# One-2-3-45/One-2-3-45

Hardware: AMD Instinct MI355X
Metric: rays/sec + mesh-extract wall-clock per scene (8x256^2 views, 128^3 vol) (higher is better)
Workload: dtype f32 (matrix products as 3 f16 MFMAs on split operands, fp32 accumulate); 1 GPU; BASELINE config 2: 1 scene/GPU/step (a different seeded scene every step), 8 views 256x256, 128^3 volume, 262144 rays (64+64 samples), mesh grid 256^3; whole scene pass per step; views=8, volume=128, rays=262144, mesh_res=256, parallelism=scenes x1, precision=f16x3

## Files before the change

include/o2345.h:

```cpp
#ifndef O2345_H
#define O2345_H
#include <stddef.h>
#include <stdint.h>
#ifdef __cplusplus
extern "C" {
#endif

const char* o2345_last_error(void);
int o2345_version(void);
size_t o2345_render_io_size(void);
int o2345_render_io_layout(size_t* offsets_host, int n);
const char* o2345_knobs(void);

size_t o2345_costvol_workspace_bytes(int dx, int dy, int dz);
int o2345_costvol_index(const float* proj, int V, int H, int W, int dx, int dy, int dz, float voxel_size,
                        const float* origin_host, int min_views, uint8_t* cnt, int32_t* row_of_voxel, int32_t* coords,
                        int32_t* n_rows_dev, void* workspace, size_t workspace_bytes, void* stream);
int o2345_costvol_gather(const float* feats_nhwc, const float* proj, int V, int H, int W, int C, int dx, int dy, int dz,
                         float voxel_size, const float* origin_host, const uint8_t* cnt, const int32_t* coords,
                         int n_rows, float* out_rows, void* stream);
int o2345_nchw_to_nhwc(const float* in, float* out, int V, int C, int H, int W, void* stream);

int o2345_fpn_level(const float* fine, int c_in, const float* coarse, const float* weight, const float* bias, int V, int H, int W,
                    float* out, void* stream);
// ... 103 lines not shown
    float inv_s, alpha_inter_ratio, background;
    float weight_cull;
    float* mid_z; float* dists; float* pm; float* sdf; float* grad; float* rgb; uint8_t* nviews;
    float* color; float* depth; float* weights; float* cdf; float* weights_sum; float* weights_max; float* depth_var;
    float* alpha_sum; float* grad_err; uint8_t* color_mask;
    float* z_vals;
    float* scalars;
    unsigned long long* color_stats;
} O2345RenderIO;
size_t o2345_list_sort_workspace_bytes(long long n_max, int V);
int o2345_list_sort_by_visibility(const float* pts, const int32_t* list, const int32_t* count_dev, long long n_max, const float* proj, int V, int H, int W,
                                  int32_t* list_out, uint32_t* keys_out, void* workspace, size_t workspace_bytes, void* stream);
size_t o2345_render_workspace_bytes(int R, int n_samples, int n_importance, int V);
int o2345_render_rays(const O2345RenderIO* io, void* workspace, size_t workspace_bytes, void* stream);

int o2345_camera_terms(const float* intrinsics, const float* w2cs, int V, float* proj_out, float* cam_pos_out, void* stream);

int o2345_pack_color_maps(const float* feat_nchw, const float* color_nchw, int V, int H, int W, float* out_nhwc64,
                          void* stream);
int o2345_view_count(const float* pts, long long n, const float* maskvol, int D, const float* proj, int V, int H, int W,
                     uint8_t* out, void* stream);
int o2345_view_count_unlisted(const float* pts, long long n, const float* skip_if_positive, const float* maskvol, int D, const float* proj,
                              int V, int H, int W, uint8_t* out, void* stream);
int o2345_color_mfma_blob_floats(void);
int o2345_color_points_mfma(const float* blob, const float* vol_cl, const float* maskvol, int D, const float* cmaps,
                            const float* proj, const float* cam_pos, int V, int H, int W, const float* pts,
                            const int32_t* index, const int32_t* n_dev, long long n, const float* query_cam,
                            const float* normals, float* out_rgb, uint8_t* out_nviews, unsigned long long* stats_dev, void* stream);
int o2345_color_x3_blob_floats(void);
int o2345_color_points_x3(const float* blob, const float* vol_cl, const float* maskvol, int D, const float* cmaps,
                          const float* proj, const float* cam_pos, int V, int H, int W, const float* pts,
                          const int32_t* index, const int32_t* n_dev, long long n, const float* query_cam,
                          const float* normals, float* out_rgb, uint8_t* out_nviews, unsigned long long* stats_dev, void* stream);
int o2345_project_features(const float* vol_cl, const float* maskvol, int D, const float* cmaps, const float* proj, const float* cam_pos, int V,
                           int H, int W, const float* pts, long long P, const float* query_cam, const float* normals, float* geometry_feat,
                           float* rgb_feat, float* ray_diff, float* mask, void* stream);
int o2345_color_from_features(const float* blob, int x3, const float* geometry_feat, const float* rgb_feat, const float* ray_diff,
                              const float* mask, int V, long long P, float* out_rgb, uint8_t* out_nviews, void* stream);

size_t o2345_mc_workspace_bytes(int n0, int n1, int n2);
int o2345_marching_cubes_count(const float* u, int n0, int n1, int n2, double iso, void* workspace,
                               size_t workspace_bytes, long long* nv_host, long long* nt_host, void* stream);
int o2345_marching_cubes_emit(const float* u, int n0, int n1, int n2, double iso, void* workspace, double* verts,
                              void* tris, int index_bytes, void* stream);

size_t o2345_mesh_components_workspace_bytes(long long nv, long long nt);
int o2345_mesh_components_count(const void* tris, int index_bytes, long long nv, long long nt, long long min_faces, int keep_largest, void* workspace,
                                size_t workspace_bytes, int* labels, long long* n_components_host, long long* n_components_kept_host,
                                long long* nv_kept_host, long long* nt_kept_host, void* stream);
int o2345_mesh_components_emit(const double* verts, const void* tris, int index_bytes, long long nv, long long nt, void* workspace, double* verts_out,
                               void* tris_out, int* kept_out, void* stream);

size_t o2345_mesh_adjacency_workspace_bytes(long long nv, long long nt);
int o2345_mesh_adjacency_count(const void* tris, int index_bytes, long long nv, long long nt, void* workspace, size_t workspace_bytes,
                               long long* n_entries_host, void* stream);
int o2345_mesh_adjacency_emit(void* workspace, long long nv, int* offsets, int* neighbours, unsigned char* boundary, void* stream);
int o2345_mesh_smooth(const double* verts_in, long long nv, const int* offsets, const int* neighbours, const unsigned char* boundary_or_null, int iterations,
                      double lam, double mu, double* verts_tmp, double* verts_out, void* stream);

size_t o2345_mesh_decimate_workspace_bytes(long long nv, long long nt);
int o2345_mesh_decimate_count(const double* verts, const void* tris, int index_bytes, long long nv, long long nt, double cell, void* workspace,
                              size_t workspace_bytes, long long* n_clusters_host, long long* nv_out_host, long long* nt_out_host,
                              long long* n_degenerate_host, long long* n_duplicate_host, void* stream);
int o2345_mesh_decimate_emit(const double* verts, const void* tris, int index_bytes, long long nv, long long nt, void* workspace, double* verts_out,
                             void* tris_out, int* cluster, void* stream);

// ... 66 lines not shown
```

one-2-3-45_amd/csrc/api.cpp:

```cpp
#include <stdarg.h>
#include <stdio.h>
#include "common.h"

namespace o2345 {
static thread_local char g_err[512] = "";
void set_error(const char* fmt, ...) {
    va_list ap;
    va_start(ap, fmt);
    vsnprintf(g_err, sizeof g_err, fmt, ap);
    va_end(ap);
}
}

#include <stddef.h>

namespace o2345 {
int preload_costvol();
int preload_sparse();
int preload_sparse_mfma();
int preload_sdf_mlp();
int preload_sdf_mlp_x3();
int preload_render();
int preload_list_sort();
int preload_color_maps();
// ... 15 lines not shown
extern "C" {
const char* o2345_last_error(void) { return o2345::g_err; }
int o2345_version(void) { return 210; }

int o2345_preload(void) {
    int e, bad = 0;
    if ((e = o2345::preload_costvol())) bad = e;
    if ((e = o2345::preload_sparse())) bad = e;
    if ((e = o2345::preload_sparse_mfma())) bad = e;
    if ((e = o2345::preload_sdf_mlp())) bad = e;
    if ((e = o2345::preload_sdf_mlp_x3())) bad = e;
    if ((e = o2345::preload_render())) bad = e;
    if ((e = o2345::preload_list_sort())) bad = e;
    if ((e = o2345::preload_color_maps())) bad = e;
    if ((e = o2345::preload_color_pts())) bad = e;
    if ((e = o2345::preload_mcubes())) bad = e;
    if ((e = o2345::preload_mesh_components())) bad = e;
    if ((e = o2345::preload_mesh_smooth())) bad = e;
    if ((e = o2345::preload_mesh_decimate())) bad = e;
    if ((e = o2345::preload_mesh_project())) bad = e;
    if ((e = o2345::preload_mesh_pack())) bad = e;
    if ((e = o2345::preload_mesh_export())) bad = e;
    if ((e = o2345::preload_mesh_texture())) bad = e;
    if ((e = o2345::preload_mesh_distance())) bad = e;
    if ((e = o2345::preload_surface_trace())) bad = e;
    if ((e = o2345::preload_featmaps())) bad = e;
    if ((e = o2345::preload_convnet())) bad = e;
    O2345_REQUIRE(bad == 0, "preload: hipFuncGetAttributes failed (%s)", hipGetErrorString((hipError_t)bad));
    return 0;
}

const char* o2345_knobs(void) {
    static const struct Text { char s[160]; Text() { const o2345::Knobs& k = o2345::knobs();
        snprintf(s, sizeof s, "list_sort=%d sparse_brick=%d flat_sched=%d color_tiles=%d color_sched=%d ray_stream_min=%lld", k.list_sort, k.sparse_brick, k.flat_sched,
                 k.color_tiles, k.color_sched, k.ray_stream_min); } } t;
    return t.s;
}

size_t o2345_render_io_size(void) { return sizeof(O2345RenderIO); }
int o2345_render_io_layout(size_t* offsets_host, int n) {
#define F(name) offsetof(O2345RenderIO, name)
    static const size_t off[] = {
        F(sdf_blob), F(color_x3_blob), F(color_mfma_blob), F(vol_cl), F(maskvol), F(cmaps), F(proj), F(cam_pos), F(D), F(V), F(H), F(W),
        F(rays_o), F(rays_d), F(near_ray), F(far_ray), F(query_cam), F(t_rand), F(R), F(n_samples), F(n_importance), F(sdf_mode), F(segment_rays),
        F(near), F(far), F(sample_dist), F(inv_s), F(alpha_inter_ratio), F(background), F(weight_cull),
        F(mid_z), F(dists), F(pm), F(sdf), F(grad), F(rgb), F(nviews), F(color), F(depth), F(weights), F(cdf), F(weights_sum), F(weights_max),
        F(depth_var), F(alpha_sum), F(grad_err), F(color_mask), F(z_vals), F(scalars), F(color_stats)};
#undef F
    const int nf = (int)(sizeof off / sizeof off[0]);
    for (int i = 0; i < n && i < nf && offsets_host; ++i) offsets_host[i] = off[i];
    return nf;
}
}
```

one-2-3-45_amd/csrc/color_mfma.hip:

```cpp
#include "color_net.h"

namespace o2345 {

#ifdef O2345_TILES_KERNEL
template <int G, bool X3>
__global__ __launch_bounds__(768) void k_color_mfma(ColorMArgs a) {
    extern __shared__ __attribute__((aligned(16))) float lds[];
    constexpr int PPT = 32 / G;
    constexpr int OPV = 64 / G;
    constexpr int PST = 2 * 64 + 4;
    constexpr int SB = PPT * PST;
    constexpr int TOTAL = X3 ? CX_TOTAL : CM_TOTAL;
    constexpr int TAIL = X3 ? CX_A_END - CM_BIAS0 : 0;
    for (int i = threadIdx.x * 4; i < TOTAL; i += blockDim.x * 4)
        *reinterpret_cast<float4*>(lds + i) = *reinterpret_cast<const float4*>(a.blob + i);
    __syncthreads();
    const int lane = threadIdx.x & 63, j = lane & 31, h = lane >> 5, ptl = j / G, v = j % G;
    const int wave = threadIdx.x >> 6, nwave = blockDim.x >> 6;
    float* sbuf = lds + TOTAL + wave * SB;
    const long long n = a.n_dev ? (long long)*a.n_dev : a.n;
    const float m1 = X3 ? opaque_minus_one() : -1.f;
    const float s_abs = fabsf(lds[TAIL + CM_S]) * LOG2E;
    const int base_prio = (a.sched & 1) ? (wave >> 2) : 0;
    if (a.sched & 1) set_wave_prio(base_prio);
// ... 79 lines not shown
                for (int r = 0; r < 16; ++r) {
                    const int nidx = 32 * b + (r & 3) + 8 * (r >> 2) + 4 * h;
                    acc[b][r] += s0[nidx] + s0[64 + nidx];
                }
            __builtin_amdgcn_wave_barrier();
        }
        float score = view_network<X3>(acc, rf, g.rd, wgt, m, m1, lds, TAIL, lds + TAIL + CM_S, lane, h);
        if (m == 0.f) score = -1e9f;
        if (!view_ok) score = -INFINITY;
        const float smax = gmax<G>(score);
        const float ex = view_ok ? __builtin_amdgcn_exp2f(score - smax) : 0.f;
        const float bw = ex * crcp(gsum<G>(ex));
        const float bwn = bw * LN2;
        const float c0 = gsum<G>(rgb0 * bwn), c1 = gsum<G>(rgb1 * bwn), c2 = gsum<G>(rgb2 * bwn);
        const float nv = gsum<G>(m);
        if (live && v == 0 && h == 0) {
            a.out_rgb[3 * slot] = c0; a.out_rgb[3 * slot + 1] = c1; a.out_rgb[3 * slot + 2] = c2;
            if (a.out_nviews) a.out_nviews[slot] = (uint8_t)(nv + 0.5f);
        }
    }
}

#endif

}

using namespace o2345;

extern "C" {

int o2345_color_mfma_blob_floats(void) { return CM_TOTAL2; }
int o2345_color_x3_blob_floats(void) { return CX_TOTAL2; }

static int color_points(int x3, const float* blob, const float* vol_cl, const float* maskvol, int D, const float* cmaps, const float* proj,
                        const float* cam_pos, int V, int H, int W, const float* pts, const int32_t* index, const int32_t* n_dev, long long n,
                        const float* query_cam, const float* normals, float* out_rgb, uint8_t* out_nviews, unsigned long long* stats_dev, void* stream) {
    O2345_REQUIRE(blob && vol_cl && maskvol && cmaps && proj && cam_pos && pts && out_rgb, "color_points: null pointer");
    O2345_REQUIRE((query_cam != nullptr) != (normals != nullptr), "color_points: give exactly one of query_cam / normals");
    O2345_REQUIRE(V >= 1 && V <= 255, "color_points: V must be in [1,255] (valid-view counts are stored as uint8; got %d)", V);
    if (n <= 0 && !n_dev) return 0;
    ColorMArgs a{blob, vol_cl, maskvol, D, cmaps, proj, cam_pos, V, H, W, pts, index, n_dev, n, query_cam, normals, out_rgb, out_nviews};
    a.sched = color_sched_mode();
    a.stats = stats_dev;
#ifdef O2345_TILES_KERNEL
    if (knobs().color_tiles && V <= 32) {
        int G = 4;
        while (G < V) G <<= 1;
        const int threads = 768, ppt = 32 / G;
        const unsigned grid = network_grid(n, n_dev, threads, ppt);
        const size_t lds = (size_t)((x3 ? CX_TOTAL : CM_TOTAL) + (threads / 64) * ppt * (2 * 64 + 4)) * sizeof(float);
        hipStream_t s = (hipStream_t)stream;
#define O2345_CM_CASE(GG, XX)                                                                                              \
    if (G == GG && (x3 != 0) == XX) {                                                                                      \
        O2345_ENSURE_LDS((k_color_mfma<GG, XX>), lds);                                                                     \
        hipLaunchKernelGGL((k_color_mfma<GG, XX>), dim3(grid), dim3(threads), lds, s, a);                                  \
    }
        O2345_CM_CASE(4, false) O2345_CM_CASE(8, false) O2345_CM_CASE(16, false) O2345_CM_CASE(32, false)
        O2345_CM_CASE(4, true) O2345_CM_CASE(8, true) O2345_CM_CASE(16, true) O2345_CM_CASE(32, true)
#undef O2345_CM_CASE
        return check_launch("color_points (tiles kernel)");
    }
#endif
    return color_pts_launch(a, x3, false, "color_points (points-as-columns kernel)", stream);
}

int o2345_color_points_mfma(const float* blob, const float* vol_cl, const float* maskvol, int D, const float* cmaps,
                            const float* proj, const float* cam_pos, int V, int H, int W, const float* pts,
                            const int32_t* index, const int32_t* n_dev, long long n, const float* query_cam,
                            const float* normals, float* out_rgb, uint8_t* out_nviews, unsigned long long* stats_dev, void* stream) {
    return color_points(0, blob, vol_cl, maskvol, D, cmaps, proj, cam_pos, V, H, W, pts, index, n_dev, n, query_cam, normals, out_rgb, out_nviews, stats_dev, stream);
}
int o2345_color_points_x3(const float* blob, const float* vol_cl, const float* maskvol, int D, const float* cmaps,
                          const float* proj, const float* cam_pos, int V, int H, int W, const float* pts,
                          const int32_t* index, const int32_t* n_dev, long long n, const float* query_cam,
                          const float* normals, float* out_rgb, uint8_t* out_nviews, unsigned long long* stats_dev, void* stream) {
    return color_points(1, blob, vol_cl, maskvol, D, cmaps, proj, cam_pos, V, H, W, pts, index, n_dev, n, query_cam, normals, out_rgb, out_nviews, stats_dev, stream);
}

int o2345_project_features(const float* vol_cl, const float* maskvol, int D, const float* cmaps, const float* proj, const float* cam_pos, int V, int H,
                           int W, const float* pts, long long P, const float* query_cam, const float* normals, float* geometry_feat, float* rgb_feat,
                           float* ray_diff, float* mask, void* stream) {
    O2345_REQUIRE(vol_cl && maskvol && cmaps && proj && cam_pos && pts && geometry_feat && rgb_feat && ray_diff && mask, "project_features: null pointer");
    O2345_REQUIRE((query_cam != nullptr) != (normals != nullptr), "project_features: give exactly one of query_cam / normals");
    O2345_REQUIRE(V >= 1 && V <= 255 && P >= 0 && P * V < (1ll << 33), "project_features: bad sizes (V in [1,255])");
    if (P == 0) return 0;
    const ColorMArgs a{nullptr, vol_cl, maskvol, D, cmaps, proj, cam_pos, V, H, W, pts, nullptr, nullptr, P, query_cam, normals, nullptr, nullptr};
    return project_features_launch(a, geometry_feat, rgb_feat, ray_diff, mask, stream);
}

int o2345_color_from_features(const float* blob, int x3, const float* geometry_feat, const float* rgb_feat, const float* ray_diff, const float* mask,
                              int V, long long P, float* out_rgb, uint8_t* out_nviews, void* stream) {
    O2345_REQUIRE(blob && geometry_feat && rgb_feat && ray_diff && mask && out_rgb, "color_from_features: null pointer");
    O2345_REQUIRE(V >= 1 && V <= 255 && P >= 0, "color_from_features: bad sizes (V in [1,255]: valid-view counts are stored as uint8)");
    if (P == 0) return 0;
    ColorMArgs a{};
    a.blob = blob; a.V = V; a.n = P; a.out_rgb = out_rgb; a.out_nviews = out_nviews;
    a.f_geo = geometry_feat; a.f_rgb = rgb_feat; a.f_rdiff = ray_diff; a.f_mask = mask;
    return color_pts_launch(a, x3, true, "color_from_features", stream);
}

}
```

one-2-3-45_amd/csrc/color_net.h:

```cpp
#pragma once
#include "common.h"
#include "geom_math.h"
#include "split_f16.h"

namespace o2345 {

#define MFMA32(a, b, c) __builtin_amdgcn_mfma_f32_32x32x2f32((a), (b), (c), 0, 0, 0)

constexpr int CM_A_RD0 = 0;
constexpr int CM_A_RD1 = CM_A_RD0 + 1 * 2 * 64;
constexpr int CM_A_B0 = CM_A_RD1 + 2 * 8 * 64;
constexpr int CM_A_B1 = CM_A_B0 + 2 * 32 * 64;
constexpr int CM_A_V0 = CM_A_B1 + 32 * 64;
constexpr int CM_A_V1 = CM_A_V0 + 16 * 64;
constexpr int CM_A_V20 = CM_A_V1 + 16 * 64;
constexpr int CM_A_R0 = CM_A_V20 + 16 * 64;
constexpr int CM_A_R1 = CM_A_R0 + 19 * 64;
constexpr int CM_BIAS0 = CM_A_R1 + 8 * 64;
constexpr int CM_B_RD0 = CM_BIAS0, CM_B_RD1 = CM_B_RD0 + 32, CM_B_B0 = CM_B_RD1 + 64, CM_B_B1 = CM_B_B0 + 64,
              CM_B_V0 = CM_B_B1 + 32, CM_B_V1 = CM_B_V0 + 32, CM_B_V20 = CM_B_V1 + 32, CM_B_R0 = CM_B_V20 + 32,
              CM_B_R1 = CM_B_R0 + 32, CM_V_V1X = CM_B_R1 + 32, CM_V_V21 = CM_V_V1X + 32, CM_V_R2 = CM_V_V21 + 32;
constexpr int CM_W_S = CM_V_R2 + 32;
constexpr int CM_S = CM_W_S + 144 * 64;
constexpr int CM_TOTAL = CM_S + 4;
constexpr int CX_A_RD0 = 0;
constexpr int CX_A_RD1 = CX_A_RD0 + 1 * 1 * 512;
constexpr int CX_A_B0 = CX_A_RD1 + 2 * 1 * 512;
constexpr int CX_A_B1 = CX_A_B0 + 2 * 4 * 512;
constexpr int CX_A_V0 = CX_A_B1 + 4 * 512;
constexpr int CX_A_V1 = CX_A_V0 + 2 * 512;
constexpr int CX_A_V20 = CX_A_V1 + 2 * 512;
constexpr int CX_A_R0 = CX_A_V20 + 2 * 512;
constexpr int CX_A_R1 = CX_A_R0 + 3 * 512;
constexpr int CX_A_END = CX_A_R1 + 1 * 512;
constexpr int CX_TOTAL = CX_A_END + (CM_TOTAL - CM_BIAS0);
constexpr int CM_A_S = CM_TOTAL;
constexpr int CM_TOTAL2 = CM_A_S + 2 * 72 * 64;
constexpr int CX_A_S = CX_TOTAL;
constexpr int CX_TOTAL2 = CX_A_S + 2 * 9 * 512;

struct ColorMArgs {
    const float* blob;
    const float* vol_cl; const float* maskvol; int D;
    const float* cmaps; const float* proj; const float* cam_pos; int V, H, W_img;
    const float* pts; const int* index; const int* n_dev; long long n;
    const float* query_cam; const float* normals;
    float* out_rgb; uint8_t* out_nviews;
    const float* f_geo;
    const float* f_rgb;
    const float* f_rdiff;
    const float* f_mask;
    unsigned long long* stats;
    int sched;
};

inline int color_sched_mode() { return knobs().color_sched; }
#if defined(__HIPCC__)
__device__ __forceinline__ void set_wave_prio(int p) {
    switch (p) {
        case 0: __builtin_amdgcn_s_setprio(0); break;
        case 1: __builtin_amdgcn_s_setprio(1); break;
        case 2: __builtin_amdgcn_s_setprio(2); break;
        default: __builtin_amdgcn_s_setprio(3); break;
    }
}
#endif

constexpr float LOG2E = 1.44269504088896340736f, LN2 = 0.69314718055994530942f;
__device__ __forceinline__ float celu(float y) {
    const float t = __builtin_amdgcn_fmed3f(__builtin_amdgcn_exp2f(y), 0.f, 1.f);
    return fmaxf(y, fmaf(t, LOG2E, -LOG2E));
}
typedef float f32x2 __attribute__((ext_vector_type(2)));
__device__ __forceinline__ f32x2 celu2(float y0, float y1) {
    f32x2 t;
    t[0] = __builtin_amdgcn_fmed3f(__builtin_amdgcn_exp2f(y0), 0.f, 1.f);
    t[1] = __builtin_amdgcn_fmed3f(__builtin_amdgcn_exp2f(y1), 0.f, 1.f);
    const f32x2 e = __builtin_elementwise_fma(t, f32x2{LOG2E, LOG2E}, f32x2{-LOG2E, -LOG2E});
    return f32x2{fmaxf(y0, e[0]), fmaxf(y1, e[1])};
}
__device__ __forceinline__ float crcp(float x) { return __builtin_amdgcn_rcpf(x); }
__device__ __forceinline__ float csigm(float z) { return crcp(1.f + __builtin_amdgcn_exp2f(-z)); }

template <int NB, int NST, int N>
__device__ __forceinline__ void cm_run(f32x16 (&acc)[NB], const float* A , int step0, const float (&b)[N]) {
    float cur[NB], nxt[NB];
// ... 274 lines not shown
```

one-2-3-45_amd/csrc/color_pts.hip:

```cpp
#include "color_net.h"

namespace o2345 {

__device__ __forceinline__ ViewGeom feat_geom(const ColorMArgs& a, int v, long long slot, float s_abs) {
    ViewGeom g;
    const float4 rd = *reinterpret_cast<const float4*>(a.f_rdiff + ((size_t)v * a.n + slot) * 4);
    g.rd[0] = rd.x; g.rd[1] = rd.y; g.rd[2] = rd.z; g.rd[3] = rd.w;
    g.e = __builtin_amdgcn_exp2f(s_abs * (rd.w - 1.f));
    g.m = a.f_mask[(size_t)v * a.n + slot] != 0.f ? 1.f : 0.f;
    g.gx = g.gy = 0.f;
    return g;
}
__device__ __forceinline__ void load_feats(const ColorMArgs& a, int h, int v, long long slot, float (&rf)[32]) {
    const float* src = a.f_rgb + ((size_t)v * a.n + slot) * 59 + 32 * h;
#pragma unroll
    for (int c = 0; c < 32; ++c) rf[c] = (h == 0 || c < 27) ? src[(h == 0 || c < 27) ? c : 0] * LOG2E : 0.f;
}

template <bool FEATS>
__device__ __forceinline__ void pixel_floats(const ColorMArgs& a, int h, int v, long long slot, const ViewGeom& g, int base_prio, float (&rf)[32]) {
    if constexpr (FEATS) load_feats(a, h, v, slot, rf);
    else {
        if (a.sched & 2) set_wave_prio(3);
        gather_now(a, h, v, g, rf);
// ... 34 lines not shown
#pragma unroll
    for (int nb = 0; nb < NB; ++nb) cur[nb] = fetch(nb, 0);
#pragma unroll
    for (int r = 0; r < N; ++r) {
        if (r + 1 < N) {
#pragma unroll
            for (int nb = 0; nb < NB; ++nb) nxt[nb] = fetch(nb, r + 1);
        }
#pragma unroll
        for (int nb = 0; nb < NB; ++nb) acc[nb] = MFMA32(cur[nb], b[r], acc[nb]);
#pragma unroll
        for (int nb = 0; nb < NB; ++nb) cur[nb] = nxt[nb];
        __builtin_amdgcn_sched_barrier(0);
    }
}

__device__ __forceinline__ void sh_store(float4* slot, const f32x16 (&sh)[2]) {
#pragma unroll
    for (int nb = 0; nb < 2; ++nb)
#pragma unroll
        for (int q = 0; q < 4; ++q) slot[(nb * 4 + q) * 64] = make_float4(sh[nb][4 * q], sh[nb][4 * q + 1], sh[nb][4 * q + 2], sh[nb][4 * q + 3]);
}
__device__ __forceinline__ void sh_load(f32x16 (&acc)[2], const float4* slot) {
#pragma unroll
    for (int nb = 0; nb < 2; ++nb)
#pragma unroll
        for (int q = 0; q < 4; ++q) {
            const float4 t = slot[(nb * 4 + q) * 64];
            acc[nb][4 * q] = t.x; acc[nb][4 * q + 1] = t.y; acc[nb][4 * q + 2] = t.z; acc[nb][4 * q + 3] = t.w;
        }
}

constexpr int CP_THREADS = 768;
constexpr int CP_SH_FLOATS = 2 * 16 * 64;
constexpr size_t color_pts_lds_bytes(int x3) {
    return (size_t)((x3 ? CX_A_END + CM_W_S - CM_BIAS0 : CM_W_S) + 4 + (CP_THREADS / 64) * CP_SH_FLOATS) * sizeof(float);
}
static_assert(color_pts_lds_bytes(1) <= 160 * 1024 && color_pts_lds_bytes(0) <= 160 * 1024, "k_color_pts: LDS of a CU exceeded");
template <bool X3, bool FEATS>
__global__ __launch_bounds__(CP_THREADS) void k_color_pts(ColorMArgs a) {
    extern __shared__ __attribute__((aligned(16))) float lds[];
    constexpr int HEAD = X3 ? (CX_A_END + CM_W_S - CM_BIAS0) : CM_W_S;
    constexpr int SRC_S = X3 ? (CX_TOTAL - 4) : CM_S;
    constexpr int TAIL = X3 ? CX_A_END - CM_BIAS0 : 0;
    constexpr int L_S = HEAD, L_SH = HEAD + 4;
    for (int i = threadIdx.x * 4; i < HEAD; i += blockDim.x * 4)
        *reinterpret_cast<float4*>(lds + i) = *reinterpret_cast<const float4*>(a.blob + i);
    if (threadIdx.x == 0) *reinterpret_cast<float4*>(lds + L_S) = *reinterpret_cast<const float4*>(a.blob + SRC_S);
    __syncthreads();
    const int lane = threadIdx.x & 63, j = lane & 31, h = lane >> 5;
    const int wave = threadIdx.x >> 6, nwave = blockDim.x >> 6;
    float4* const sh_slot = reinterpret_cast<float4*>(lds + L_SH + wave * CP_SH_FLOATS) + lane;
    const long long n = a.n_dev ? (long long)*a.n_dev : a.n;
    const float m1 = X3 ? opaque_minus_one() : -1.f;
    const float s_abs = fabsf(lds[L_S]) * LOG2E;
    const int V = a.V;
    const bool skip_views = V <= 64 && !(a.sched & 4);
    const bool skip_zero = skip_views && !(a.sched & 16);
    const int base_prio = (a.sched & 1) ? (wave >> 2) : 0;
    if (a.sched & 1) set_wave_prio(base_prio);
    const TileSched ts = (a.sched & 8) ? TileSched{(long long)blockIdx.x * nwave + wave, (n + 31) / 32, (long long)gridDim.x * nwave}
                                       : tile_schedule(n, 32, wave, nwave);
    unsigned st_a = 0, st_b = 0, st_t = 0, st_full = 0;
    for (long long tile = ts.first; tile < ts.end; tile += ts.stride) {
        const long long i = tile * 32 + j;
        const bool live = i < n;
        const long long slot = live ? (a.index ? (long long)a.index[i] : i) : 0;
        const float px = (live && !FEATS) ? a.pts[3 * slot] : 0.f, py = (live && !FEATS) ? a.pts[3 * slot + 1] : 0.f,
                    pz = (live && !FEATS) ? a.pts[3 * slot + 2] : 0.f;
        float bs[72];
        bool gvalid;
        if constexpr (FEATS) {
            const float4* g4 = reinterpret_cast<const float4*>(a.f_geo + (size_t)slot * 16) + 2 * h;
            const float4 t0 = g4[0], t1 = g4[1];
            bs[0] = t0.x; bs[1] = t0.y; bs[2] = t0.z; bs[3] = t0.w; bs[4] = t1.x; bs[5] = t1.y; bs[6] = t1.z; bs[7] = t1.w;
            gvalid = true;
        } else {
#pragma unroll
            for (int c = 0; c < 8; ++c) bs[c] = 0.f;
            const float msum = trilinear_taps(px, py, pz, a.D, a.maskvol, [&](size_t vox, float w) {
                fma_rows<2>(reinterpret_cast<const float4*>(a.vol_cl + vox * 16) + 2 * h, w, bs);
            });
            gvalid = point_valid(px, py, pz, msum);
        }
        float qx = 0.f, qy = 0.f, qz = 0.f;
        if constexpr (!FEATS) query_direction(a.normals, a.query_cam, slot, px, py, pz, qx, qy, qz);
        float emin = INFINITY;
        for (int v = 0; v < V; ++v) {
            if constexpr (FEATS) {
                emin = fminf(emin, __builtin_amdgcn_exp2f(s_abs * (a.f_rdiff[((size_t)v * a.n + slot) * 4 + 3] - 1.f)));
                continue;
            }
            const float sx = a.cam_pos[3 * v] - px, sy = a.cam_pos[3 * v + 1] - py, sz = a.cam_pos[3 * v + 2] - pz;
            const float rsn = crcp(sqrtf(sx * sx + sy * sy + sz * sz) + 1e-6f);
            const float dot = qx * (sx * rsn) + qy * (sy * rsn) + qz * (sz * rsn);
            emin = fminf(emin, __builtin_amdgcn_exp2f(s_abs * (dot - 1.f)));
        }
// ... 151 lines not shown
```

one-2-3-45_amd/csrc/common.h:

```cpp
#pragma once
#include "../../include/o2345.h"
#include <atomic>
#include <cstdlib>
#include <hip/hip_runtime.h>
#include <stdint.h>
#include <stdio.h>

#define O2345_HD __host__ __device__ __forceinline__

namespace o2345 {

void set_error(const char* fmt, ...);

inline int check_launch(const char* what) {
    hipError_t e = hipGetLastError();
    if (e != hipSuccess) {
        set_error("%s: %s", what, hipGetErrorString(e));
        return -2;
    }
    return 0;
}

#define O2345_REQUIRE(cond, ...)            \
    do {                                    \
// ... 28 lines not shown

__device__ __forceinline__ int lane_id() { return __lane_id(); }

__device__ __forceinline__ int wave_prefix(bool pred, int& total) {
    unsigned long long m = __ballot(pred);
    total = __popcll(m);
    return __popcll(m & ((1ull << lane_id()) - 1ull));
}

template <int NWAVES>
__device__ __forceinline__ int block_prefix(bool pred, int* lds_wave_tot , int& block_total) {
    int wtot;
    int p = wave_prefix(pred, wtot);
    const int w = threadIdx.x >> 6;
    if (lane_id() == 0) lds_wave_tot[w] = wtot;
    __syncthreads();
    int base = 0, tot = 0;
#pragma unroll
    for (int i = 0; i < NWAVES; ++i) {
        int t = lds_wave_tot[i];
        if (i < w) base += t;
        tot += t;
    }
    block_total = tot;
    __syncthreads();
    return base + p;
}


struct Knobs {
    bool list_sort, sparse_brick, flat_sched, color_tiles;
    int color_sched;
    long long ray_stream_min;
};
inline const Knobs& knobs() {
    static const Knobs k = [] {
        auto is = [](const char* name, char c) { const char* e = getenv(name); return e && e[0] == c; };
        const char* cs = getenv("O2345_COLOR_SCHED");
        const char* rs = getenv("O2345_RAY_STREAM_MIN");
        return Knobs{!is("O2345_LIST_SORT", '0'), !is("O2345_SPARSE_BRICK", '0'), is("O2345_FLAT_SCHED", '1'), is("O2345_COLOR_KERNEL", 't'), cs ? atoi(cs) : 10,
                     rs ? atoll(rs) : 4096};
    }();
    return k;
}

struct MaxLds {
    std::atomic<int> cur[64];
    MaxLds() { for (auto& c : cur) c.store(0, std::memory_order_relaxed); }
    hipError_t ensure(const void* func, size_t bytes) {
        int dev = 0;
        if (hipGetDevice(&dev) != hipSuccess || dev < 0 || dev >= 64) return hipFuncSetAttribute(func, hipFuncAttributeMaxDynamicSharedMemorySize, (int)bytes);
        if ((int)bytes <= cur[dev].load(std::memory_order_acquire)) return hipSuccess;
        const hipError_t e = hipFuncSetAttribute(func, hipFuncAttributeMaxDynamicSharedMemorySize, (int)bytes);
        if (e == hipSuccess) cur[dev].store((int)bytes, std::memory_order_release);
        return e;
    }
};
#define O2345_ENSURE_LDS(kernel, bytes)                                                   \
    do {                                                                                  \
        static o2345::MaxLds max_lds_;                                                    \
        O2345_HIP(max_lds_.ensure((const void*)(kernel), (size_t)(bytes)));               \
    } while (0)

inline unsigned persistent_grid(long long want, int n_cu) {
    unsigned g = (unsigned)(want < n_cu ? want : n_cu);
    if (knobs().flat_sched && g > 8 && (g & 7) == 0) --g;
    return g;
}

inline unsigned network_grid(long long n, const void* n_dev, int threads, int units_per_wave) {
    const int n_cu = cu_count();
    const long long per_block = (long long)(threads / 64) * units_per_wave;
    return persistent_grid(n_dev ? n_cu : (n + per_block - 1) / per_block, n_cu);
}

#if defined(__HIPCC__)
struct TileSched { long long first, end, stride; };
__device__ __forceinline__ TileSched tile_schedule(long long n_units, int units_per_tile, int wave, int nwave) {
    const long long ntiles = (n_units + units_per_tile - 1) / units_per_tile;
    if ((gridDim.x & 7) == 0) {
        const int xcd = blockIdx.x & 7, slot = blockIdx.x >> 3, per_xcd = gridDim.x >> 3;
        const long long chunk = (ntiles + 7) / 8, lo = xcd * chunk, hi = lo + chunk;
        return {lo + (long long)slot * nwave + wave, hi < ntiles ? hi : ntiles, (long long)per_xcd * nwave};
    }
    return {(long long)blockIdx.x * nwave + wave, ntiles, (long long)gridDim.x * nwave};
}
#endif

}
```

one-2-3-45_amd/csrc/render.hip:

```cpp
#include "common.h"
#include "render_math.h"

namespace o2345 {

enum RenderCounter {
    RC_ROUND = 0,
    RC_FINAL = 4,
    RC_CULLED = 5,
    RC_DONE = 8,
    RC_CLEARED = 16,
    RC_RESERVED = 64
};

__global__ __launch_bounds__(256) void k_ray_coarse(RayGeom g, float near, float far, const float* __restrict__ near_ray,
                                                    const float* __restrict__ far_ray, int S, const float* __restrict__ t_rand,
                                                    float* __restrict__ z, float* __restrict__ pts, const float* __restrict__ maskvol, int D,
                                                    uint8_t* __restrict__ msk, int* __restrict__ counters) {
    if (counters && blockIdx.x == 0 && threadIdx.x < RC_CLEARED) counters[threadIdx.x] = 0;
    const long long p = (long long)blockIdx.x * 256 + threadIdx.x;
    if (p >= (long long)S * g.R) return;
    const int s = (int)(p / g.R), r = (int)(p % g.R);
    if (near_ray) { near = near_ray[r]; far = far_ray[r]; }
    float zz = near + (far - near) * linspace_at(0.f, 1.f, S, s);
    if (t_rand) {
        const float zp = near + (far - near) * linspace_at(0.f, 1.f, S, s > 0 ? s - 1 : 0);
        const float zn = near + (far - near) * linspace_at(0.f, 1.f, S, s < S - 1 ? s + 1 : S - 1);
        const float lower = s > 0 ? 0.5f * (zz + zp) : zz;
        const float upper = s < S - 1 ? 0.5f * (zn + zz) : zz;
        zz = lower + (upper - lower) * t_rand[(long long)r * S + s];
    }
    z[p] = zz;
    float x, y, w;
    ray_point(g, r, zz, x, y, w);
    pts[3 * p] = x; pts[3 * p + 1] = y; pts[3 * p + 2] = w;
    if (msk) msk[p] = mask_at(maskvol, D, x, y, w) > 0.f ? 1 : 0;
}

__device__ __forceinline__ unsigned long long lanes_below() { return (1ull << (threadIdx.x & 63)) - 1ull; }
__device__ __forceinline__ int reserve_slots(int* __restrict__ count, int n, int* __restrict__ seg_cnt, int ray0, int seg_rays) {
    const int base = atomicAdd(count, n);
    if (seg_cnt) atomicAdd(seg_cnt + ray0 / seg_rays, n);
    return base;
}
__device__ __forceinline__ void append_lane(bool valid, int slot, int* __restrict__ list, int* __restrict__ count, int* __restrict__ seg_cnt = nullptr,
                                            int ray0 = 0, int seg_rays = 0) {
// ... 752 lines not shown
    const bool sorts = render_sorts_list(R, NS, NIMP, io->V);
    int* slist = lay.at<int>(workspace, lay.sorted_list);
    auto sort_list = [&](const int* in, const int* n_dev) {
        return o2345_list_sort_by_visibility(fpts, in, n_dev, (long long)(S * RR), io->proj, io->V, io->H, io->W, slist, nullptr, lay.at<void>(workspace, lay.sort_ws),
                                             lay.sort_ws.bytes, stream);
    };
    const int* clist = list;
    const int* ccount = count;
    const float* counted_elsewhere = io->pm;
    if (!cull && sorts) {
        if ((rc = sort_list(list, count))) return rc;
        list = slist; clist = slist;
    }
    if ((rc = sdf_eval(2, fpts, list, count, 0, io->sdf, io->grad))) return rc;
    if (cull) {
        int* list2 = lay.at<int>(workspace, lay.cull_list);
        int* count2 = counters + RC_CULLED;
        float* keep = sdf;
        const size_t lds = group_lds_bytes(CULL_ARRAYS, (int)S);
        if (use_group_form(R, lds))
            hipLaunchKernelGGL(k_ray_cull_group, dim3(cdiv(R, GR)), dim3(64), lds, s, ra.g, (int)S, io->dists, io->pm, io->sdf, io->grad, io->inv_s, io->alpha_inter_ratio,
                               io->weight_cull, keep, io->rgb, list2, count2);
        else
            hipLaunchKernelGGL(k_ray_cull, dim3(cdiv(R, 256)), dim3(256), 0, s, ra.g, (int)S, io->dists, io->pm, io->sdf, io->grad, io->inv_s, io->alpha_inter_ratio,
                               io->weight_cull, keep, io->rgb, list2, count2);
        if ((rc = check_launch("ray_cull"))) return rc;
        clist = list2; ccount = count2; counted_elsewhere = keep;
        if (sorts) {
            if ((rc = sort_list(list2, count2))) return rc;
            clist = slist;
        }
    }
    if ((rc = o2345_view_count_unlisted(fpts, (long long)S * R, counted_elsewhere, io->maskvol, io->D, io->proj, io->V, io->H, io->W, io->nviews, stream))) return rc;
    const auto color_points = io->color_x3_blob ? o2345_color_points_x3 : o2345_color_points_mfma;
    rc = color_points(io->color_x3_blob ? io->color_x3_blob : io->color_mfma_blob, io->vol_cl, io->maskvol, io->D, io->cmaps, io->proj, io->cam_pos, io->V, io->H, io->W, fpts, clist,
                      ccount, 0, io->query_cam, nullptr, io->rgb, io->nviews, io->color_stats, stream);
    if (rc) return rc;
    if ((rc = o2345_ray_composite(io->rays_o, io->rays_d, R, (int)S, io->mid_z, io->dists, io->pm, io->sdf, io->grad, io->rgb, io->nviews, io->inv_s, io->alpha_inter_ratio, io->background,
                                  io->color, io->depth, io->weights, io->cdf, io->weights_sum, io->weights_max, io->depth_var, io->alpha_sum, io->grad_err, io->color_mask, stream))) return rc;
    if (io->scalars) hipLaunchKernelGGL(k_ray_scalars, dim3(G ? n_seg : 1), dim3(1024), 0, s, R, (int)S, io->alpha_sum, io->grad_err, G ? segc + (size_t)4 * n_seg : count,
                                        io->scalars, G);
    if (io->z_vals) O2345_HIP(hipMemcpyAsync(io->z_vals, z, S * RR * sizeof(float), hipMemcpyDeviceToDevice, s));
    return check_launch("render_rays");
}

}

namespace o2345 {
int preload_render() {
    hipFuncAttributes at;
    return (int)hipFuncGetAttributes(&at, (const void*)(k_quirk_min2));
}
}
```

one-2-3-45_amd/ops.py:

```python
import ctypes
import functools
from collections import namedtuple
import threading

import numpy as np
import torch

from . import _lib, config, mesh_io


call = _lib.call


def _first_cuda_tensor(objs):
    for o in objs:
        if torch.is_tensor(o):
            if o.is_cuda:
                return o
        elif isinstance(o, dict):
            t = _first_cuda_tensor(o.values())
            if t is not None:
                return t
    return None

# ... 396 lines not shown
             res.get("lat"), res.get("grad"))
    return res


def sdf_grid_active_points(device):
    with torch.cuda.device(device):
        ws = _workspace(None, torch.device(device), "sdf_grid_sparse")
    return None if ws is None else int(ws[:4].view(torch.int32).item())


@_on_device
def pack_color_maps(feat_nchw, color_nchw):
    V, _, H, W = feat_nchw.shape
    out = torch.empty(V, H, W, 64, dtype=torch.float32, device=feat_nchw.device)
    call("o2345_pack_color_maps", feat_nchw, color_nchw, V, H, W, out)
    return out


@_on_device
def camera_terms(intrinsics, w2cs):
    V = intrinsics.shape[0]
    if tuple(intrinsics.shape) != (V, 3, 3) or tuple(w2cs.shape) != (V, 4, 4):
        raise ValueError(f"camera_terms: intrinsics [V,3,3] and w2cs [V,4,4] expected, got {tuple(intrinsics.shape)}, {tuple(w2cs.shape)}")
    proj = torch.empty(V, 3, 4, dtype=torch.float32, device=w2cs.device)
    cam = torch.empty(V, 3, dtype=torch.float32, device=w2cs.device)
    call("o2345_camera_terms", _f(intrinsics), _f(w2cs), V, proj, cam)
    return proj, cam


def color_stats_buffer(device):
    return torch.zeros(4, dtype=torch.int64, device=device)


def color_stats_read(buf):
    out = [int(x) for x in buf.cpu().tolist()]
    return dict(pairs_pooling=out[0], pairs_network=out[1], tiles=out[2], tiles_all_views=out[3])


@_on_device
def color_points(blob, vol_cl, maskvol, cmaps, proj, cam_pos, pts, query_cam=None, normals=None, index=None, n_dev=None,
                 want_nviews=True, mfma="x3", stats=None):
    if mfma is False or mfma is None:
        raise ValueError("color_points: the pure-VALU colour kernel was removed in ABI 2.0; pass mfma='x3' (split-f16) or mfma=True (fp32 MFMA)")
    V, H, W, _ = cmaps.shape
    P = pts.shape[0]
    n = P if index is None else index.shape[0]
    rgb = torch.zeros(P, 3, dtype=torch.float32, device=pts.device)
    nv = torch.zeros(P, dtype=torch.uint8, device=pts.device) if want_nviews else None
    if P == 0 or (n == 0 and n_dev is None):
        return rgb, nv
    call("o2345_color_points_x3" if mfma == "x3" else "o2345_color_points_mfma", blob, vol_cl, maskvol, vol_cl.shape[0], cmaps, proj, cam_pos,
         V, H, W, pts, index, n_dev, n, query_cam, normals, rgb, nv, stats)
    return rgb, nv


@_on_device
def project_features(vol_cl, maskvol, cmaps, proj, cam_pos, pts, query_cam=None, normals=None):
    V, H, W, _ = cmaps.shape
    P = pts.shape[0]
    dev = pts.device
    geo = torch.empty(P, 16, dtype=torch.float32, device=dev)
    rf = torch.empty(V, P, 59, dtype=torch.float32, device=dev)
    rd = torch.empty(V, P, 4, dtype=torch.float32, device=dev)
    m = torch.empty(V, P, dtype=torch.float32, device=dev)
    call("o2345_project_features", vol_cl, maskvol, vol_cl.shape[0], cmaps, proj, cam_pos, V, H, W, pts, P, query_cam, normals, geo, rf, rd, m)
    return geo, rf, rd, m


@_on_device
def color_from_features(blob, geometry_feat, rgb_feat, ray_diff, mask, x3=True, want_nviews=True):
    V, P, C = rgb_feat.shape
    if C != 59 or tuple(geometry_feat.shape) != (P, 16) or tuple(ray_diff.shape) != (V, P, 4) or tuple(mask.shape) != (V, P):
        raise ValueError(f"color_from_features: expected geometry_feat [P,16], rgb_feat [V,P,59], ray_diff [V,P,4], mask [V,P]; got "
                         f"{tuple(geometry_feat.shape)}, {tuple(rgb_feat.shape)}, {tuple(ray_diff.shape)}, {tuple(mask.shape)}")
    rgb = torch.empty(P, 3, dtype=torch.float32, device=rgb_feat.device)
    nv = torch.empty(P, dtype=torch.uint8, device=rgb_feat.device) if want_nviews else None
    if P:
        call("o2345_color_from_features", blob, int(bool(x3)), _f(geometry_feat), _f(rgb_feat), _f(ray_diff), _f(mask), V, P, rgb, nv)
    return rgb, nv


@_on_device
def view_count(pts, maskvol, D, proj, V, H, W):
    out = torch.empty(pts.shape[0], dtype=torch.uint8, device=pts.device)
    call("o2345_view_count", pts, pts.shape[0], maskvol, D, proj, V, H, W, out)
# ... 688 lines not shown
```

Before: 4.680 million rays/s.

## Add atomic tile queue for dynamic load balancing in colour-points kernel

Adds a dynamic tile queue to the colour-points MFMA kernel. A fraction of the tiles is handed out from 8 per-XCD atomic heads instead of a fixed strided schedule. With the default share shift of 0, every tile is claimed dynamically. The queue heads live in the render counter block, which k_ray_coarse clears, and the queue is on by default through a new knob. The aim is to even out per-wave work when tiles differ in cost (views skipped, masked points), at the price of one atomic per tile and the loss of the static per-XCD chunking.

Result: faster. 4.903 million rays/s (median of 6 runs) (+4.8%).

```diff
diff --git a/include/o2345.h b/include/o2345.h
--- a/include/o2345.h
+++ b/include/o2345.h
@@ -159,6 +159,14 @@
                           const float* proj, const float* cam_pos, int V, int H, int W, const float* pts,
                           const int32_t* index, const int32_t* n_dev, long long n, const float* query_cam,
                           const float* normals, float* out_rgb, uint8_t* out_nviews, unsigned long long* stats_dev, void* stream);
+int o2345_color_points_mfma_q(const float* blob, const float* vol_cl, const float* maskvol, int D, const float* cmaps,
+                              const float* proj, const float* cam_pos, int V, int H, int W, const float* pts,
+                              const int32_t* index, const int32_t* n_dev, long long n, const float* query_cam,
+                              const float* normals, float* out_rgb, uint8_t* out_nviews, unsigned long long* stats_dev, int32_t* tile_queue, void* stream);
+int o2345_color_points_x3_q(const float* blob, const float* vol_cl, const float* maskvol, int D, const float* cmaps,
+                            const float* proj, const float* cam_pos, int V, int H, int W, const float* pts,
+                            const int32_t* index, const int32_t* n_dev, long long n, const float* query_cam,
+                            const float* normals, float* out_rgb, uint8_t* out_nviews, unsigned long long* stats_dev, int32_t* tile_queue, void* stream);
 int o2345_project_features(const float* vol_cl, const float* maskvol, int D, const float* cmaps, const float* proj, const float* cam_pos, int V,
                            int H, int W, const float* pts, long long P, const float* query_cam, const float* normals, float* geometry_feat,
                            float* rgb_feat, float* ray_diff, float* mask, void* stream);
diff --git a/one-2-3-45_amd/csrc/api.cpp b/one-2-3-45_amd/csrc/api.cpp
--- a/one-2-3-45_amd/csrc/api.cpp
+++ b/one-2-3-45_amd/csrc/api.cpp
@@ -71,8 +71,8 @@
 
 const char* o2345_knobs(void) {
     static const struct Text { char s[160]; Text() { const o2345::Knobs& k = o2345::knobs();
-        snprintf(s, sizeof s, "list_sort=%d sparse_brick=%d flat_sched=%d color_tiles=%d color_sched=%d ray_stream_min=%lld", k.list_sort, k.sparse_brick, k.flat_sched,
-                 k.color_tiles, k.color_sched, k.ray_stream_min); } } t;
+        snprintf(s, sizeof s, "list_sort=%d sparse_brick=%d flat_sched=%d color_tiles=%d color_sched=%d ray_stream_min=%lld tile_queue=%d", k.list_sort, k.sparse_brick,
+                 k.flat_sched, k.color_tiles, k.color_sched, k.ray_stream_min, k.tile_queue); } } t;
     return t.s;
 }
 
diff --git a/one-2-3-45_amd/csrc/color_mfma.hip b/one-2-3-45_amd/csrc/color_mfma.hip
--- a/one-2-3-45_amd/csrc/color_mfma.hip
+++ b/one-2-3-45_amd/csrc/color_mfma.hip
@@ -135,16 +135,21 @@
 int o2345_color_mfma_blob_floats(void) { return CM_TOTAL2; }
 int o2345_color_x3_blob_floats(void) { return CX_TOTAL2; }
 
-static int color_points(int x3, const float* blob, const float* vol_cl, const float* maskvol, int D, const float* cmaps, const float* proj,
-                        const float* cam_pos, int V, int H, int W, const float* pts, const int32_t* index, const int32_t* n_dev, long long n,
-                        const float* query_cam, const float* normals, float* out_rgb, uint8_t* out_nviews, unsigned long long* stats_dev, void* stream) {
+}
+
+int o2345::color_points_launch(int x3, const float* blob, const float* vol_cl, const float* maskvol, int D, const float* cmaps, const float* proj,
+                               const float* cam_pos, int V, int H, int W, const float* pts, const int32_t* index, const int32_t* n_dev, long long n,
+                               const float* query_cam, const float* normals, float* out_rgb, uint8_t* out_nviews, unsigned long long* stats_dev,
+                               int32_t* tile_queue, void* stream) {
     O2345_REQUIRE(blob && vol_cl && maskvol && cmaps && proj && cam_pos && pts && out_rgb, "color_points: null pointer");
     O2345_REQUIRE((query_cam != nullptr) != (normals != nullptr), "color_points: give exactly one of query_cam / normals");
     O2345_REQUIRE(V >= 1 && V <= 255, "color_points: V must be in [1,255] (valid-view counts are stored as uint8; got %d)", V);
     if (n <= 0 && !n_dev) return 0;
+    O2345_REQUIRE(!tile_queue || n <= TQ_MAX_TILES * 32, "color_points: a tile queue indexes at most %lld tiles", TQ_MAX_TILES);
     ColorMArgs a{blob, vol_cl, maskvol, D, cmaps, proj, cam_pos, V, H, W, pts, index, n_dev, n, query_cam, normals, out_rgb, out_nviews};
     a.sched = color_sched_mode();
     a.stats = stats_dev;
+    a.tile_queue = tile_queue;
 #ifdef O2345_TILES_KERNEL
     if (knobs().color_tiles && V <= 32) {
         int G = 4;
@@ -167,17 +172,43 @@
     return color_pts_launch(a, x3, false, "color_points (points-as-columns kernel)", stream);
 }
 
+extern "C" {
+
+static int color_points_q(int x3, const float* blob, const float* vol_cl, const float* maskvol, int D, const float* cmaps, const float* proj,
+                          const float* cam_pos, int V, int H, int W, const float* pts, const int32_t* index, const int32_t* n_dev, long long n,
+                          const float* query_cam, const float* normals, float* out_rgb, uint8_t* out_nviews, unsigned long long* stats_dev,
+                          int32_t* tile_queue, void* stream) {
+    O2345_REQUIRE(tile_queue, "color_points_q: null tile queue");
+    O2345_HIP(hipMemsetAsync(tile_queue, 0, TQ_HEADS * sizeof(int32_t), (hipStream_t)stream));
+    return color_points_launch(x3, blob, vol_cl, maskvol, D, cmaps, proj, cam_pos, V, H, W, pts, index, n_dev, n, query_cam, normals, out_rgb, out_nviews, stats_dev,
+                               tile_queue, stream);
+}
+int o2345_color_points_x3_q(const float* blob, const float* vol_cl, const float* maskvol, int D, const float* cmaps,
+                            const float* proj, const float* cam_pos, int V, int H, int W, const float* pts,
+                            const int32_t* index, const int32_t* n_dev, long long n, const float* query_cam,
+                            const float* normals, float* out_rgb, uint8_t* out_nviews, unsigned long long* stats_dev, int32_t* tile_queue, void* stream) {
+    return color_points_q(1, blob, vol_cl, maskvol, D, cmaps, proj, cam_pos, V, H, W, pts, index, n_dev, n, query_cam, normals, out_rgb, out_nviews, stats_dev,
+                          tile_queue, stream);
+}
+int o2345_color_points_mfma_q(const float* blob, const float* vol_cl, const float* maskvol, int D, const float* cmaps,
+                              const float* proj, const float* cam_pos, int V, int H, int W, const float* pts,
+                              const int32_t* index, const int32_t* n_dev, long long n, const float* query_cam,
+                              const float* normals, float* out_rgb, uint8_t* out_nviews, unsigned long long* stats_dev, int32_t* tile_queue, void* stream) {
+    return color_points_q(0, blob, vol_cl, maskvol, D, cmaps, proj, cam_pos, V, H, W, pts, index, n_dev, n, query_cam, normals, out_rgb, out_nviews, stats_dev,
+                          tile_queue, stream);
+}
+
 int o2345_color_points_mfma(const float* blob, const float* vol_cl, const float* maskvol, int D, const float* cmaps,
                             const float* proj, const float* cam_pos, int V, int H, int W, const float* pts,
                             const int32_t* index, const int32_t* n_dev, long long n, const float* query_cam,
                             const float* normals, float* out_rgb, uint8_t* out_nviews, unsigned long long* stats_dev, void* stream) {
-    return color_points(0, blob, vol_cl, maskvol, D, cmaps, proj, cam_pos, V, H, W, pts, index, n_dev, n, query_cam, normals, out_rgb, out_nviews, stats_dev, stream);
+    return color_points_launch(0, blob, vol_cl, maskvol, D, cmaps, proj, cam_pos, V, H, W, pts, index, n_dev, n, query_cam, normals, out_rgb, out_nviews, stats_dev, nullptr, stream);
 }
 int o2345_color_points_x3(const float* blob, const float* vol_cl, const float* maskvol, int D, const float* cmaps,
                           const float* proj, const float* cam_pos, int V, int H, int W, const float* pts,
                           const int32_t* index, const int32_t* n_dev, long long n, const float* query_cam,
                           const float* normals, float* out_rgb, uint8_t* out_nviews, unsigned long long* stats_dev, void* stream) {
-    return color_points(1, blob, vol_cl, maskvol, D, cmaps, proj, cam_pos, V, H, W, pts, index, n_dev, n, query_cam, normals, out_rgb, out_nviews, stats_dev, stream);
+    return color_points_launch(1, blob, vol_cl, maskvol, D, cmaps, proj, cam_pos, V, H, W, pts, index, n_dev, n, query_cam, normals, out_rgb, out_nviews, stats_dev, nullptr, stream);
 }
 
 int o2345_project_features(const float* vol_cl, const float* maskvol, int D, const float* cmaps, const float* proj, const float* cam_pos, int V, int H,
diff --git a/one-2-3-45_amd/csrc/color_net.h b/one-2-3-45_amd/csrc/color_net.h
--- a/one-2-3-45_amd/csrc/color_net.h
+++ b/one-2-3-45_amd/csrc/color_net.h
@@ -52,6 +52,7 @@
     const float* f_mask;
     unsigned long long* stats;
     int sched;
+    int* tile_queue;
 };
 
 inline int color_sched_mode() { return knobs().color_sched; }
diff --git a/one-2-3-45_amd/csrc/color_pts.hip b/one-2-3-45_amd/csrc/color_pts.hip
--- a/one-2-3-45_amd/csrc/color_pts.hip
+++ b/one-2-3-45_amd/csrc/color_pts.hip
@@ -90,6 +90,10 @@
 }
 
 constexpr int CP_THREADS = 768;
+#ifndef O2345_CP_TQ_SHARE_SHIFT
+#define O2345_CP_TQ_SHARE_SHIFT 0
+#endif
+constexpr int CP_TQ_SHARE_SHIFT = O2345_CP_TQ_SHARE_SHIFT, CP_TQ_CLAIM = 1;
 constexpr int CP_SH_FLOATS = 2 * 16 * 64;
 constexpr size_t color_pts_lds_bytes(int x3) {
     return (size_t)((x3 ? CX_A_END + CM_W_S - CM_BIAS0 : CM_W_S) + 4 + (CP_THREADS / 64) * CP_SH_FLOATS) * sizeof(float);
@@ -117,10 +121,12 @@
     const bool skip_zero = skip_views && !(a.sched & 16);
     const int base_prio = (a.sched & 1) ? (wave >> 2) : 0;
     if (a.sched & 1) set_wave_prio(base_prio);
-    const TileSched ts = (a.sched & 8) ? TileSched{(long long)blockIdx.x * nwave + wave, (n + 31) / 32, (long long)gridDim.x * nwave}
-                                       : tile_schedule(n, 32, wave, nwave);
+    const TileQueue tq = tile_queue_split((n + 31) / 32, (long long)gridDim.x * nwave, CP_TQ_SHARE_SHIFT, a.tile_queue != nullptr);
+    const TileSched ts = (a.sched & 8) ? tile_schedule_flat_at(tq.n_static, blockIdx.x, gridDim.x, wave, nwave) : tile_schedule_tiles(tq.n_static, wave, nwave);
+    const auto static_end = [&](long long n_static) { return (a.sched & 8) ? n_static : tile_schedule_tiles(n_static, wave, nwave).end; };
+    TileCursor cur;
     unsigned st_a = 0, st_b = 0, st_t = 0, st_full = 0;
-    for (long long tile = ts.first; tile < ts.end; tile += ts.stride) {
+    for (long long tile = tile_first<CP_TQ_CLAIM>(cur, ts, tq, a.tile_queue); tile >= 0; tile = tile_next<CP_TQ_CLAIM>(cur, tile, (n + 31) / 32, a.tile_queue, static_end)) {
         const long long i = tile * 32 + j;
         const bool live = i < n;
         const long long slot = live ? (a.index ? (long long)a.index[i] : i) : 0;
diff --git a/one-2-3-45_amd/csrc/common.h b/one-2-3-45_amd/csrc/common.h
--- a/one-2-3-45_amd/csrc/common.h
+++ b/one-2-3-45_amd/csrc/common.h
@@ -84,6 +84,7 @@
     bool list_sort, sparse_brick, flat_sched, color_tiles;
     int color_sched;
     long long ray_stream_min;
+    bool tile_queue;
 };
 inline const Knobs& knobs() {
     static const Knobs k = [] {
@@ -91,7 +92,7 @@
         const char* cs = getenv("O2345_COLOR_SCHED");
         const char* rs = getenv("O2345_RAY_STREAM_MIN");
         return Knobs{!is("O2345_LIST_SORT", '0'), !is("O2345_SPARSE_BRICK", '0'), is("O2345_FLAT_SCHED", '1'), is("O2345_COLOR_KERNEL", 't'), cs ? atoi(cs) : 10,
-                     rs ? atoll(rs) : 4096};
+                     rs ? atoll(rs) : 4096, !is("O2345_TILE_QUEUE", '0')};
     }();
     return k;
 }
@@ -126,16 +127,92 @@
     return persistent_grid(n_dev ? n_cu : (n + per_block - 1) / per_block, n_cu);
 }
 
-#if defined(__HIPCC__)
 struct TileSched { long long first, end, stride; };
-__device__ __forceinline__ TileSched tile_schedule(long long n_units, int units_per_tile, int wave, int nwave) {
-    const long long ntiles = (n_units + units_per_tile - 1) / units_per_tile;
-    if ((gridDim.x & 7) == 0) {
-        const int xcd = blockIdx.x & 7, slot = blockIdx.x >> 3, per_xcd = gridDim.x >> 3;
+O2345_HD TileSched tile_schedule_flat_at(long long ntiles, int block, int grid, int wave, int nwave) {
+    return {(long long)block * nwave + wave, ntiles, (long long)grid * nwave};
+}
+O2345_HD TileSched tile_schedule_at(long long ntiles, int block, int grid, int wave, int nwave) {
+    if ((grid & 7) == 0) {
+        const int xcd = block & 7, slot = block >> 3, per_xcd = grid >> 3;
         const long long chunk = (ntiles + 7) / 8, lo = xcd * chunk, hi = lo + chunk;
         return {lo + (long long)slot * nwave + wave, hi < ntiles ? hi : ntiles, (long long)per_xcd * nwave};
     }
-    return {(long long)blockIdx.x * nwave + wave, ntiles, (long long)gridDim.x * nwave};
+    return tile_schedule_flat_at(ntiles, block, grid, wave, nwave);
+}
+
+constexpr int TQ_HEADS = 8;
+constexpr long long TQ_MAX_TILES = (1ll << 31) - 64;
+struct TileQueue { long long n_static; int n_dyn, per_head; };
+O2345_HD TileQueue tile_queue_of(long long ntiles, int n_dyn) { return {ntiles - n_dyn, n_dyn, (n_dyn + TQ_HEADS - 1) / TQ_HEADS}; }
+O2345_HD TileQueue tile_queue_split(long long ntiles, long long total_waves, int share_shift, bool queued) {
+    if (!queued) return {ntiles, 0, 0};
+    long long ns = ntiles - (ntiles >> share_shift);
+    ns -= ns % total_waves;
+    return tile_queue_of(ntiles, (int)(ntiles - ns));
+}
+O2345_HD int tile_queue_lo(const TileQueue& q, int head) {
+    const long long lo = (long long)head * q.per_head;
+    return lo < q.n_dyn ? (int)lo : q.n_dyn;
+}
+struct TileWalk { int head, left; };
+O2345_HD TileWalk tile_walk_begin(int block) { return {block & (TQ_HEADS - 1), TQ_HEADS}; }
+O2345_HD long long tile_walk_take(const TileQueue& q, TileWalk& w, int claimed, int C, long long& end) {
+    const long long t = (long long)tile_queue_lo(q, w.head) + claimed, hi = tile_queue_lo(q, w.head + 1);
+    if (t < hi) {
+        end = q.n_static + (t + C < hi ? t + C : hi);
+        return q.n_static + t;
+    }
+    w.head = (w.head + 1) & (TQ_HEADS - 1);
+    --w.left;
+    return -1;
+}
+
+int color_points_launch(int x3, const float* blob, const float* vol_cl, const float* maskvol, int D, const float* cmaps, const float* proj,
+                        const float* cam_pos, int V, int H, int W, const float* pts, const int32_t* index, const int32_t* n_dev, long long n,
+                        const float* query_cam, const float* normals, float* out_rgb, uint8_t* out_nviews, unsigned long long* stats_dev, int32_t* tile_queue,
+                        void* stream);
+
+#if defined(__HIPCC__)
+__device__ __forceinline__ TileSched tile_schedule_tiles(long long ntiles, int wave, int nwave) {
+    return tile_schedule_at(ntiles, blockIdx.x, gridDim.x, wave, nwave);
+}
+__device__ __forceinline__ TileSched tile_schedule(long long n_units, int units_per_tile, int wave, int nwave) {
+    return tile_schedule_tiles((n_units + units_per_tile - 1) / units_per_tile, wave, nwave);
+}
+
+struct TileCursor { int stride, n_dyn, walk; long long claim_end; };
+template <int C>
+__device__ __forceinline__ long long tile_claim(TileCursor& c, const TileQueue& q, int* heads) {
+    c.stride = 0;
+    TileWalk w{c.walk & 15, c.walk >> 4};
+    long long first = -1;
+    while (first < 0 && w.left > 0) {
+        int t = 0;
+        if (lane_id() == 0) t = __hip_atomic_fetch_add(heads + w.head, C, __ATOMIC_RELAXED, __HIP_MEMORY_SCOPE_AGENT);
+        first = tile_walk_take(q, w, __builtin_amdgcn_readfirstlane(t), C, c.claim_end);
+    }
+    c.walk = w.head | w.left << 4;
+    return first;
+}
+template <int C>
+__device__ __forceinline__ long long tile_first(TileCursor& c, const TileSched& ts, const TileQueue& q, int* heads) {
+    const TileWalk w = tile_walk_begin(blockIdx.x);
+    c = TileCursor{(int)ts.stride, q.n_dyn, w.head | w.left << 4, 0};
+    if (ts.first < ts.end) return ts.first;
+    return heads ? tile_claim<C>(c, q, heads) : -1;
+}
+template <int C, class StaticEnd>
+__device__ __forceinline__ long long tile_next(TileCursor& c, long long tile, long long ntiles, int* heads, StaticEnd&& static_end) {
+    asm volatile("" : "+s"(c.n_dyn));
+    const TileQueue q = tile_queue_of(ntiles, c.n_dyn);
+    if (c.stride) {
+        tile += c.stride;
+        if (tile < static_end(q.n_static)) return tile;
+        if (!heads) return -1;
+    } else if (C > 1 && tile + 1 < c.claim_end) {
+        return tile + 1;
+    }
+    return tile_claim<C>(c, q, heads);
 }
 #endif
 
diff --git a/one-2-3-45_amd/csrc/render.hip b/one-2-3-45_amd/csrc/render.hip
--- a/one-2-3-45_amd/csrc/render.hip
+++ b/one-2-3-45_amd/csrc/render.hip
@@ -8,9 +8,11 @@
     RC_FINAL = 4,
     RC_CULLED = 5,
     RC_DONE = 8,
-    RC_CLEARED = 16,
+    RC_QUEUE = 16,
+    RC_CLEARED = 24,
     RC_RESERVED = 64
 };
+static_assert(RC_QUEUE + TQ_HEADS <= RC_CLEARED && RC_CLEARED <= RC_RESERVED && RC_CLEARED <= 256, "k_ray_coarse clears the counters with one 256-thread workgroup");
 
 __global__ __launch_bounds__(256) void k_ray_coarse(RayGeom g, float near, float far, const float* __restrict__ near_ray,
                                                     const float* __restrict__ far_ray, int S, const float* __restrict__ t_rand,
@@ -829,9 +831,9 @@
         }
     }
     if ((rc = o2345_view_count_unlisted(fpts, (long long)S * R, counted_elsewhere, io->maskvol, io->D, io->proj, io->V, io->H, io->W, io->nviews, stream))) return rc;
-    const auto color_points = io->color_x3_blob ? o2345_color_points_x3 : o2345_color_points_mfma;
-    rc = color_points(io->color_x3_blob ? io->color_x3_blob : io->color_mfma_blob, io->vol_cl, io->maskvol, io->D, io->cmaps, io->proj, io->cam_pos, io->V, io->H, io->W, fpts, clist,
-                      ccount, 0, io->query_cam, nullptr, io->rgb, io->nviews, io->color_stats, stream);
+    rc = color_points_launch(io->color_x3_blob != nullptr, io->color_x3_blob ? io->color_x3_blob : io->color_mfma_blob, io->vol_cl, io->maskvol, io->D, io->cmaps, io->proj,
+                             io->cam_pos, io->V, io->H, io->W, fpts, clist, ccount, 0, io->query_cam, nullptr, io->rgb, io->nviews, io->color_stats,
+                             knobs().tile_queue ? counters + RC_QUEUE : nullptr, stream);
     if (rc) return rc;
     if ((rc = o2345_ray_composite(io->rays_o, io->rays_d, R, (int)S, io->mid_z, io->dists, io->pm, io->sdf, io->grad, io->rgb, io->nviews, io->inv_s, io->alpha_inter_ratio, io->background,
                                   io->color, io->depth, io->weights, io->cdf, io->weights_sum, io->weights_max, io->depth_var, io->alpha_sum, io->grad_err, io->color_mask, stream))) return rc;
diff --git a/one-2-3-45_amd/ops.py b/one-2-3-45_amd/ops.py
--- a/one-2-3-45_amd/ops.py
+++ b/one-2-3-45_amd/ops.py
@@ -452,6 +452,16 @@
     return torch.zeros(4, dtype=torch.int64, device=device)
 
 
+def tile_queue_buffer(device):
+    return torch.empty(8, dtype=torch.int32, device=device)
+
+
+def _tile_queue(buf):
+    if buf.dtype != torch.int32 or buf.numel() < 8 or not buf.is_contiguous():
+        raise ValueError("tile_queue: 8 contiguous int32 on the device expected (ops.tile_queue_buffer)")
+    return buf
+
+
 def color_stats_read(buf):
     out = [int(x) for x in buf.cpu().tolist()]
     return dict(pairs_pooling=out[0], pairs_network=out[1], tiles=out[2], tiles_all_views=out[3])
@@ -459,18 +469,27 @@
 
 @_on_device
 def color_points(blob, vol_cl, maskvol, cmaps, proj, cam_pos, pts, query_cam=None, normals=None, index=None, n_dev=None,
-                 want_nviews=True, mfma="x3", stats=None):
+                 want_nviews=True, mfma="x3", stats=None, tile_queue=None, out=None):
     if mfma is False or mfma is None:
         raise ValueError("color_points: the pure-VALU colour kernel was removed in ABI 2.0; pass mfma='x3' (split-f16) or mfma=True (fp32 MFMA)")
     V, H, W, _ = cmaps.shape
     P = pts.shape[0]
     n = P if index is None else index.shape[0]
-    rgb = torch.zeros(P, 3, dtype=torch.float32, device=pts.device)
-    nv = torch.zeros(P, dtype=torch.uint8, device=pts.device) if want_nviews else None
+    if out is not None:
+        rgb, nv = out
+        if tuple(rgb.shape) != (P, 3) or rgb.dtype != torch.float32 or (nv is not None and (tuple(nv.shape) != (P,) or nv.dtype != torch.uint8)):
+            raise ValueError(f"color_points: out = (rgb [{P},3] float32, nviews [{P}] uint8 or None) expected")
+    else:
+        rgb = torch.zeros(P, 3, dtype=torch.float32, device=pts.device)
+        nv = torch.zeros(P, dtype=torch.uint8, device=pts.device) if want_nviews else None
     if P == 0 or (n == 0 and n_dev is None):
         return rgb, nv
-    call("o2345_color_points_x3" if mfma == "x3" else "o2345_color_points_mfma", blob, vol_cl, maskvol, vol_cl.shape[0], cmaps, proj, cam_pos,
-         V, H, W, pts, index, n_dev, n, query_cam, normals, rgb, nv, stats)
+    entry = "o2345_color_points_x3" if mfma == "x3" else "o2345_color_points_mfma"
+    if tile_queue is not None:
+        call(entry + "_q", blob, vol_cl, maskvol, vol_cl.shape[0], cmaps, proj, cam_pos, V, H, W, pts, index, n_dev, n, query_cam, normals, rgb, nv, stats,
+             _tile_queue(tile_queue))
+    else:
+        call(entry, blob, vol_cl, maskvol, vol_cl.shape[0], cmaps, proj, cam_pos, V, H, W, pts, index, n_dev, n, query_cam, normals, rgb, nv, stats)
     return rgb, nv
 
 
```
